# snap-research/R2L

Hardware: AMD Instinct MI355X
Metric: rays/sec (train+render) W256D88 lego@400x400 (higher is better)
Workload: dtype f32 (v_mfma_f32_32x32x2_f32: exact fp32 products and accumulate)

## Files before the change

r2l_amd/csrc/r2l_coop16.hip:

```cpp
#include "r2l_common.h"

#define C16_RAYS 16
#define C16_LD 260
#define C16_ACT_FLOATS (C16_RAYS * C16_LD)
#define C16_GROUP_BYTES (R2L_C16_GROUP_FLOATS * 4)

typedef float f32x4v __attribute__((ext_vector_type(4)));

__host__ __device__ static inline int64_t h_off_head_b() { return (int64_t)R2L_IN * R2L_W; }
__host__ __device__ static inline int64_t h_off_body_w(int layer) {
    return (int64_t)R2L_IN * R2L_W + R2L_W + (int64_t)layer * (R2L_W * R2L_W + R2L_W);
}
__host__ __device__ static inline int64_t h_off_body_b(int layer) { return h_off_body_w(layer) + R2L_W * R2L_W; }
__host__ __device__ static inline int64_t h_off_tail_w(int n_block) { return h_off_body_w(2 * n_block); }
__host__ __device__ static inline int64_t h_off_tail_b(int n_block) { return h_off_tail_w(n_block) + 3 * R2L_W; }
#define C16_BIAS_STRIDE (R2L_W * R2L_W + R2L_W)

template <int D>
struct Ring16 {
    __amdgpu_buffer_rsrc_t rsrc;
    unsigned voff;
    unsigned soff;
    f32x4 w[D][4];
    __device__ __forceinline__ f32x4 load(int t) const {
        return __builtin_bit_cast(f32x4, __builtin_amdgcn_raw_buffer_load_b128(rsrc, voff + (unsigned)t * 1024u, soff, 0));
    }
    __device__ __forceinline__ void opaque() { asm volatile("" : "+v"(voff)); }
    __device__ __forceinline__ void init(const float* stream, int64_t first_group, int lane, int wave) {
        rsrc = __builtin_amdgcn_make_buffer_rsrc(const_cast<float*>(stream), 0, 0xffffffff, 0x00020000);
        voff = (unsigned)lane * 16u + (unsigned)(4 * wave) * 1024u;
        soff = (unsigned)(first_group * C16_GROUP_BYTES);
#pragma unroll
        for (int d = 0; d < D; ++d) {
#pragma unroll
            for (int t = 0; t < 4; ++t) w[d][t] = load(t);
            soff += C16_GROUP_BYTES;
        }
    }
};

template <int SLOT, int EXTRA_RD = 0, int VPT = 0, int D>
__device__ __forceinline__ void group16(f32x4 (&acc)[4], Ring16<D>& r, const f32x4& b) {
    static_assert(SLOT >= 0 && SLOT < D, "ring slot");
    r.opaque();
#pragma unroll
    for (int e = 0; e < 3; ++e)
#pragma unroll
        for (int t = 0; t < 4; ++t) acc[t] = __builtin_amdgcn_mfma_f32_16x16x4f32(r.w[SLOT][t][e], b[e], acc[t], 0, 0, 0);
#pragma unroll
    for (int t = 0; t < 4; ++t) {
        acc[t] = __builtin_amdgcn_mfma_f32_16x16x4f32(r.w[SLOT][t][3], b[3], acc[t], 0, 0, 0);
        r.w[SLOT][t] = r.load(t);
    }
    r.soff += C16_GROUP_BYTES;
    if (EXTRA_RD > 0) __builtin_amdgcn_sched_group_barrier(0x020, EXTRA_RD, 0);
#pragma unroll
    for (int i = 0; i < 12; ++i) {
        __builtin_amdgcn_sched_group_barrier(0x008, 1, 0);
        if (VPT > 0) __builtin_amdgcn_sched_group_barrier(0x002, VPT, 0);
    }
#pragma unroll
    for (int i = 0; i < 4; ++i) {
        __builtin_amdgcn_sched_group_barrier(0x008, 1, 0);
        __builtin_amdgcn_sched_group_barrier(0x020, 1, 0);
        if (VPT > 0) __builtin_amdgcn_sched_group_barrier(0x002, VPT, 0);
    }
    __builtin_amdgcn_sched_barrier(0);
}

__device__ __forceinline__ void layer16(f32x4 (&acc)[4], const f32x4 (&bop)[16], Ring16<8>& r, const float* next_bias,
                                        f32x4 (&bn)[4]) {
#pragma unroll
    for (int t = 0; t < 4; ++t) bn[t] = *reinterpret_cast<const f32x4*>(next_bias + 16 * t);
    group16<0, 4>(acc, r, bop[0]);
    group16<1>(acc, r, bop[1]);
    group16<2>(acc, r, bop[2]);
    group16<3>(acc, r, bop[3]);
    group16<4>(acc, r, bop[4]);
    group16<5>(acc, r, bop[5]);
    group16<6>(acc, r, bop[6]);
    group16<7>(acc, r, bop[7]);
    group16<0>(acc, r, bop[8]);
    group16<1>(acc, r, bop[9]);
    group16<2>(acc, r, bop[10]);
    group16<3>(acc, r, bop[11]);
    group16<4>(acc, r, bop[12]);
    group16<5>(acc, r, bop[13]);
    group16<6>(acc, r, bop[14]);
    group16<7>(acc, r, bop[15]);
}

__device__ __forceinline__ void lds_read_bops16(const float* act, int lane, f32x4 (&bop)[16]) {
    const float* row = act + (lane & 15) * C16_LD + 4 * (lane >> 4);
#pragma unroll
    for (int G = 0; G < 16; ++G) bop[G] = *reinterpret_cast<const f32x4*>(row + 16 * G);
}
__device__ __forceinline__ void lds_write_slice16(float* act, int lane, int wave, const f32x4 (&v)[4]) {
    float* row = act + (lane & 15) * C16_LD + 64 * wave + 4 * (lane >> 4);
#pragma unroll
    for (int t = 0; t < 4; ++t) *reinterpret_cast<f32x4*>(row + 16 * t) = v[t];
}
__device__ __forceinline__ void g_store_slice16(float* base, int64_t ray, int lane, int wave, const f32x4 (&v)[4]) {
    float* row = base + ray * R2L_W + 64 * wave + 4 * (lane >> 4);
#pragma unroll
    for (int t = 0; t < 4; ++t) r2l_stash_store(row + 16 * t, v[t]);
}
__device__ __forceinline__ void g_load_slice16(const float* base, int64_t ray, int lane, int wave, f32x4 (&v)[4]) {
    const float* row = base + ray * R2L_W + 64 * wave + 4 * (lane >> 4);
#pragma unroll
    for (int t = 0; t < 4; ++t) v[t] = *reinterpret_cast<const f32x4*>(row + 16 * t);
}
__device__ __forceinline__ void rows_lds_to_global(const float* act, float* base, int64_t tile_row0, int lane, int wave) {
#pragma unroll
    for (int r = 0; r < 4; ++r) {
        const int ray = 4 * wave + r;
        const f32x4 v = *reinterpret_cast<const f32x4*>(act + ray * C16_LD + 4 * lane);
        r2l_stash_store_nt(base + (tile_row0 + ray) * R2L_W + 4 * lane, v);
    }
}
__device__ __forceinline__ float sel4(int kk, float a0, float a1, float a2, float a3) {
    const float lo = kk == 1 ? a1 : a0, hi = kk == 3 ? a3 : a2;
    return kk >= 2 ? hi : lo;
}

struct C16FwdArgs {
    const float* rays_o;
    const float* rays_d;
    const float* t_rand;
    const float* ztab;
    float c2w[12];
    int H, Wimg;
    float focal;
    const float* wstream;
    const float* params;
    int n_block;
    float* rgb;
    float* save_x;
    float* save_t;
    int64_t N;
};

template <int Gp>
__device__ __forceinline__ f32x4 trig_chunk(int kk, const float (&xb)[4]) {
    constexpr int o0 = 16 * Gp, o1 = o0 + 4, o2 = o0 + 8, o3 = o0 + 12;
    const float x = sel4(kk, xb[o0 / 20], xb[o1 / 20], xb[o2 / 20], xb[o3 / 20]);
    const float sc = sel4(kk, (float)(1 << ((o0 % 20) / 2)), (float)(1 << ((o1 % 20) / 2)), (float)(1 << ((o2 % 20) / 2)),
                          (float)(1 << ((o3 % 20) / 2)));
    f32x4 v;
    float s, c;
    r2l_sincos(x * sc, s, c);
    v[0] = s;
    v[1] = c;
    r2l_sincos(x * (sc + sc), s, c);
    v[2] = s;
    v[3] = c;
    return v;
}

template <bool POSE, bool SAVE>
__global__ __launch_bounds__(256, 1) void r2l_fwd_c16_kernel(const C16FwdArgs a) {
    __shared__ __attribute__((aligned(16))) float act[2][C16_ACT_FLOATS];
    __shared__ float tailred[4][C16_RAYS][4];
    __shared__ float zl[4][C16_RAYS][20];

    const int wave = threadIdx.x >> 6, lane = threadIdx.x & 63, j = lane & 15, kk = lane >> 4;
    const int64_t tile_row0 = (int64_t)blockIdx.x * C16_RAYS;
    const int64_t ray = tile_row0 + j;
    const bool valid = ray < a.N;
    const int64_t rc = valid ? ray : a.N - 1;
    const int64_t Np = R2L_PAD_ROWS(a.N);

    float o[3], d[3];
    if constexpr (!POSE) {
#pragma unroll
        for (int k = 0; k < 3; ++k) {
            o[k] = a.rays_o[rc * 3 + k];
            d[k] = a.rays_d[rc * 3 + k];
        }
    } else {
        const int pj = (int)(rc / a.Wimg), pi = (int)(rc % a.Wimg);
        const float dx = ((float)pi - (float)a.Wimg * 0.5f) / a.focal;
        const float dy = -(((float)pj - (float)a.H * 0.5f) / a.focal);
#pragma unroll
        for (int k = 0; k < 3; ++k) {
            d[k] = (dx * a.c2w[4 * k + 0] + dy * a.c2w[4 * k + 1]) + (-1.0f) * a.c2w[4 * k + 2];
            o[k] = a.c2w[4 * k + 3];
        }
    }
    float z[16];
#pragma unroll
    for (int q = 0; q < 4; ++q) {
        const f32x4 lo = *reinterpret_cast<const f32x4*>(a.ztab + 4 * q);
#pragma unroll
        for (int k = 0; k < 4; ++k) z[4 * q + k] = lo[k];
        if (a.t_rand != nullptr) {
            const f32x4 sp = *reinterpret_cast<const f32x4*>(a.ztab + 16 + 4 * q);
            const f32x4 u = *reinterpret_cast<const f32x4*>(a.t_rand + rc * 16 + 4 * q);
#pragma unroll
            for (int k = 0; k < 4; ++k) z[4 * q + k] = lo[k] + sp[k] * u[k];
        }
    }

    f32x4 acc[4], xo[4], x0[4], bn[4];
    {
        const float* hb = a.params + h_off_head_b() + 64 * wave + 4 * kk;
#pragma unroll
        for (int t = 0; t < 4; ++t) acc[t] = *reinterpret_cast<const f32x4*>(hb + 16 * t);
    }
    Ring16<5> r5;
    r5.init(a.wstream, 0, lane, wave);
#pragma unroll
    for (int q = 0; q < 4; ++q)
        *reinterpret_cast<f32x4*>(&zl[wave][j][4 * q]) = f32x4{z[4 * q], z[4 * q + 1], z[4 * q + 2], z[4 * q + 3]};
    auto coords = [&](int S, float (&xc)[12]) {
        const f32x4 zs = *reinterpret_cast<const f32x4*>(&zl[wave][j][4 * (S & 3)]);
#pragma unroll
        for (int i = 0; i < 12; ++i) xc[i] = o[i % 3] + d[i % 3] * zs[i / 3];
    };
    {
        float xc[12], xn[12];
        coords(0, xc);
        f32x4 cur, nxt;
        {
            const float xb[4] = {xc[0], xc[1], xc[2], xc[3]};
            cur = trig_chunk<0>(kk, xb);
        }
#define C16_HEAD_STEP(SLOT, NEXT_GP, XB)                   \
    nxt = trig_chunk<NEXT_GP>(kk, XB);                     \
    group16<SLOT, 0, 6>(acc, r5, cur);                     \
    cur = nxt;
#pragma unroll 1
        for (int S = 0; S < 4; ++S) {
            coords(S + 1, xn);
            const float b0[4] = {xc[0], xc[1], xc[2], xc[3]}, b1[4] = {xc[4], xc[5], xc[6], xc[7]};
            const float b2[4] = {xc[8], xc[9], xc[10], xc[11]}, b3[4] = {xn[0], xn[1], xn[2], xn[3]};
            C16_HEAD_STEP(0, 1, b0) C16_HEAD_STEP(1, 2, b0) C16_HEAD_STEP(2, 3, b0) C16_HEAD_STEP(3, 4, b0)
            C16_HEAD_STEP(4, 0, b1)
            C16_HEAD_STEP(0, 1, b1) C16_HEAD_STEP(1, 2, b1) C16_HEAD_STEP(2, 3, b1) C16_HEAD_STEP(3, 4, b1)
            C16_HEAD_STEP(4, 0, b2)
            C16_HEAD_STEP(0, 1, b2) C16_HEAD_STEP(1, 2, b2) C16_HEAD_STEP(2, 3, b2) C16_HEAD_STEP(3, 4, b2)
            C16_HEAD_STEP(4, 0, b3)
#pragma unroll
            for (int i = 0; i < 12; ++i) xc[i] = xn[i];
        }
#undef C16_HEAD_STEP
    }
    {
        float p[48];
#pragma unroll
        for (int c = 0; c < 48; ++c) p[c] = o[c % 3] + d[c % 3] * z[c / 3];
        f32x4 idv[3];
#pragma unroll
        for (int g = 0; g < 3; ++g)
#pragma unroll
            for (int e = 0; e < 4; ++e) idv[g][e] = sel4(kk, p[16 * g + e], p[16 * g + 4 + e], p[16 * g + 8 + e], p[16 * g + 12 + e]);
        group16<0>(acc, r5, idv[0]);
        group16<1>(acc, r5, idv[1]);
        group16<2>(acc, r5, idv[2]);
    }
#pragma unroll
    for (int t = 0; t < 4; ++t)
#pragma unroll
        for (int c = 0; c < 4; ++c) {
            xo[t][c] = fmaxf(acc[t][c], 0.f);
            x0[t][c] = xo[t][c];
        }
    lds_write_slice16(act[0], lane, wave, xo);
    Ring16<8> r8;
    r8.rsrc = r5.rsrc;
    r8.voff = r5.voff;
    r8.soff = r5.soff;
#pragma unroll
    for (int t = 0; t < 4; ++t) {
        r8.w[0][t] = r5.w[3][t];
        r8.w[1][t] = r5.w[4][t];
        r8.w[2][t] = r5.w[0][t];
        r8.w[3][t] = r5.w[1][t];
        r8.w[4][t] = r5.w[2][t];
    }
#pragma unroll
    for (int dd = 5; dd < 8; ++dd) {
#pragma unroll
        for (int t = 0; t < 4; ++t) r8.w[dd][t] = r8.load(t);
        r8.soff += C16_GROUP_BYTES;
    }

    f32x4 bop[16];
    const float* bias = a.params + h_off_body_b(0) + 64 * wave + 4 * kk;
#pragma unroll
    for (int t = 0; t < 4; ++t) bn[t] = *reinterpret_cast<const f32x4*>(bias + 16 * t);
#pragma unroll 1
    for (int b = 0; b < a.n_block; ++b) {
        __syncthreads();
        lds_read_bops16(act[0], lane, bop);
        if constexpr (SAVE) rows_lds_to_global(act[0], a.save_x + (int64_t)b * Np * R2L_W, tile_row0, lane, wave);
#pragma unroll
        for (int t = 0; t < 4; ++t) acc[t] = bn[t];
        layer16(acc, bop, r8, bias + C16_BIAS_STRIDE, bn);
#pragma unroll
        for (int t = 0; t < 4; ++t)
#pragma unroll
            for (int c = 0; c < 4; ++c) acc[t][c] = fmaxf(acc[t][c], 0.f);
        lds_write_slice16(act[1], lane, wave, acc);
        __syncthreads();
        lds_read_bops16(act[1], lane, bop);
        if constexpr (SAVE) rows_lds_to_global(act[1], a.save_t + (int64_t)b * Np * R2L_W, tile_row0, lane, wave);
#pragma unroll
        for (int t = 0; t < 4; ++t) xo[t] += bn[t];
        layer16(xo, bop, r8, b + 1 < a.n_block ? bias + 2 * C16_BIAS_STRIDE : bias, bn);
        lds_write_slice16(act[0], lane, wave, xo);
        bias += 2 * C16_BIAS_STRIDE;
    }
    if constexpr (SAVE) {
        __syncthreads();
        rows_lds_to_global(act[0], a.save_x + (int64_t)a.n_block * Np * R2L_W, tile_row0, lane, wave);
    }

    const float* tw = a.params + h_off_tail_w(a.n_block) + 64 * wave + 4 * kk;
    float p3[3] = {0.f, 0.f, 0.f};
#pragma unroll
    for (int t = 0; t < 4; ++t) {
        f32x4 wv[3];
#pragma unroll
        for (int c = 0; c < 3; ++c) wv[c] = *reinterpret_cast<const f32x4*>(tw + c * R2L_W + 16 * t);
#pragma unroll
        for (int e = 0; e < 4; ++e) {
            const float y = xo[t][e] + x0[t][e];
#pragma unroll
            for (int c = 0; c < 3; ++c) p3[c] = __builtin_fmaf(wv[c][e], y, p3[c]);
        }
    }
#pragma unroll
    for (int c = 0; c < 3; ++c) {
        p3[c] += __shfl_xor(p3[c], 16);
        p3[c] += __shfl_xor(p3[c], 32);
    }
    if (kk == 0) {
        tailred[wave][j][0] = p3[0];
        tailred[wave][j][1] = p3[1];
        tailred[wave][j][2] = p3[2];
    }
    __syncthreads();
    if (wave == 0 && kk == 0 && valid) {
#pragma unroll
        for (int c = 0; c < 3; ++c) {
            const float v = ((tailred[0][j][c] + tailred[1][j][c]) + (tailred[2][j][c] + tailred[3][j][c])) +
                            a.params[h_off_tail_b(a.n_block) + c];
            a.rgb[ray * 3 + c] = 1.0f / (1.0f + expf(-v));
        }
    }
}

struct C16BwdArgs {
    const float* rgb;
    const float* target;
    const float* drgb;
    const float* save_x;
    const float* save_t;
    const float* wstream;
    const float* params;
    int n_block;
    float grad_scale;
    float* dpre;
    float* gx;
    float* gt;
    float* sqerr_partial;
    int64_t N;
};

__device__ __forceinline__ void layer16_plain(f32x4 (&acc)[4], const f32x4 (&bop)[16], Ring16<8>& r) {
    group16<0>(acc, r, bop[0]);
    group16<1>(acc, r, bop[1]);
    group16<2>(acc, r, bop[2]);
    group16<3>(acc, r, bop[3]);
    group16<4>(acc, r, bop[4]);
    group16<5>(acc, r, bop[5]);
    group16<6>(acc, r, bop[6]);
    group16<7>(acc, r, bop[7]);
    group16<0>(acc, r, bop[8]);
    group16<1>(acc, r, bop[9]);
    group16<2>(acc, r, bop[10]);
    group16<3>(acc, r, bop[11]);
    group16<4>(acc, r, bop[12]);
    group16<5>(acc, r, bop[13]);
    group16<6>(acc, r, bop[14]);
    group16<7>(acc, r, bop[15]);
}

__global__ __launch_bounds__(256, 1) void r2l_bwd_c16_kernel(const C16BwdArgs a) {
    __shared__ __attribute__((aligned(16))) float act[2][C16_ACT_FLOATS];

    const int wave = threadIdx.x >> 6, lane = threadIdx.x & 63, j = lane & 15, kk = lane >> 4;
    const int64_t tile = blockIdx.x;
    const int64_t ray = tile * C16_RAYS + j;
    const bool valid = ray < a.N;
    const int64_t rc = valid ? ray : a.N - 1;
    const int64_t Np = R2L_PAD_ROWS(a.N);

    Ring16<8> r8;
    r8.init(a.wstream, 0, lane, wave);

    float dp[3];
#pragma unroll
    for (int c = 0; c < 3; ++c) {
        const float r = a.rgb[rc * 3 + c];
        const float dl = a.target != nullptr ? a.grad_scale * (r - a.target[rc * 3 + c]) : a.drgb[rc * 3 + c];
        dp[c] = valid ? dl * (r * (1.0f - r)) : 0.f;
    }
    if (wave == 0 && kk == 0 && valid) {
#pragma unroll
        for (int c = 0; c < 3; ++c) a.dpre[ray * 3 + c] = dp[c];
    }
    if (a.sqerr_partial != nullptr && (tile & 1) == 0 && wave == 1) {
        const int64_t r32 = tile * C16_RAYS + (lane & 31);
        float s = 0.f;
        if (a.target != nullptr && lane < 32 && r32 < a.N) {
#pragma unroll
            for (int c = 0; c < 3; ++c) {
                const float e = a.rgb[r32 * 3 + c] - a.target[r32 * 3 + c];
                s += e * e;
            }
        }
#pragma unroll
        for (int off = 32; off >= 1; off >>= 1) s += __shfl_xor(s, off);
        if (lane == 0) a.sqerr_partial[tile >> 1] = s;
    }
    f32x4 g[4], dy[4], u[4];
    {
        const float* tw = a.params + h_off_tail_w(a.n_block) + 64 * wave + 4 * kk;
#pragma unroll
        for (int t = 0; t < 4; ++t) {
            f32x4 wv[3];
#pragma unroll
            for (int c = 0; c < 3; ++c) wv[c] = *reinterpret_cast<const f32x4*>(tw + c * R2L_W + 16 * t);
#pragma unroll
            for (int e = 0; e < 4; ++e) {
                float v = wv[0][e] * dp[0];
                v = __builtin_fmaf(wv[1][e], dp[1], v);
                v = __builtin_fmaf(wv[2][e], dp[2], v);
                g[t][e] = v;
                dy[t][e] = v;
            }
        }
    }
    lds_write_slice16(act[0], lane, wave, g);

    f32x4 bop[16];
    const int64_t tile_row0 = tile * C16_RAYS;
#pragma unroll 1
    for (int b = a.n_block - 1; b >= 0; --b) {
        __syncthreads();
        lds_read_bops16(act[0], lane, bop);
        rows_lds_to_global(act[0], a.gx + (int64_t)(b + 1) * Np * R2L_W, tile_row0, lane, wave);
        f32x4 tm[4];
        g_load_slice16(a.save_t + (int64_t)b * Np * R2L_W, ray, lane, wave, tm);
#pragma unroll
        for (int t = 0; t < 4; ++t) u[t] = f32x4{0.f, 0.f, 0.f, 0.f};
        layer16_plain(u, bop, r8);
#pragma unroll
        for (int t = 0; t < 4; ++t)
#pragma unroll
            for (int c = 0; c < 4; ++c) u[t][c] = tm[t][c] > 0.f ? u[t][c] : 0.f;
        lds_write_slice16(act[1], lane, wave, u);
        __syncthreads();
        lds_read_bops16(act[1], lane, bop);
        rows_lds_to_global(act[1], a.gt + (int64_t)b * Np * R2L_W, tile_row0, lane, wave);
        layer16_plain(g, bop, r8);
        lds_write_slice16(act[0], lane, wave, g);
    }
    f32x4 xm[4];
    g_load_slice16(a.save_x, ray, lane, wave, xm);
#pragma unroll
    for (int t = 0; t < 4; ++t)
#pragma unroll
        for (int c = 0; c < 4; ++c) g[t][c] = xm[t][c] > 0.f ? g[t][c] + dy[t][c] : 0.f;
    g_store_slice16(a.gx, ray, lane, wave, g);
}

int r2l_coop16_forward(const float* rays_o, const float* rays_d, const float* t_rand, const float* ztab,
                       const float* c2w_host12, int H, int W, float focal, const float* wstream16, const float* params,
                       int n_block, float* rgb, float* save_x, float* save_t, int64_t N, hipStream_t stream) {
    C16FwdArgs a{};
    a.rays_o = rays_o; a.rays_d = rays_d; a.t_rand = t_rand; a.ztab = ztab; a.wstream = wstream16; a.params = params;
    a.n_block = n_block; a.rgb = rgb; a.save_x = save_x; a.save_t = save_t; a.N = N; a.H = H; a.Wimg = W; a.focal = focal;
    if (c2w_host12) for (int i = 0; i < 12; ++i) a.c2w[i] = c2w_host12[i];
    const dim3 grid((unsigned)(R2L_PAD_ROWS(N) / C16_RAYS)), block(256);
    if (c2w_host12) hipLaunchKernelGGL((r2l_fwd_c16_kernel<true, false>), grid, block, 0, stream, a);
    else if (save_x) hipLaunchKernelGGL((r2l_fwd_c16_kernel<false, true>), grid, block, 0, stream, a);
    else hipLaunchKernelGGL((r2l_fwd_c16_kernel<false, false>), grid, block, 0, stream, a);
    R2L_CHECK(hipGetLastError());
    return 0;
}

int r2l_coop16_backward(const float* rgb, const float* target, const float* drgb, const float* save_x,
                        const float* save_t, const float* wstream_bwd16, const float* params, int n_block,
                        float grad_scale, float* dpre, float* gx, float* gt, float* sqerr_partial, int64_t N,
                        hipStream_t stream) {
    C16BwdArgs a{};
    a.rgb = rgb; a.target = target; a.drgb = drgb; a.save_x = save_x; a.save_t = save_t; a.wstream = wstream_bwd16;
    a.params = params; a.n_block = n_block; a.grad_scale = grad_scale; a.dpre = dpre; a.gx = gx; a.gt = gt;
    a.sqerr_partial = sqerr_partial; a.N = N;
    const dim3 grid((unsigned)(R2L_PAD_ROWS(N) / C16_RAYS)), block(256);
    hipLaunchKernelGGL(r2l_bwd_c16_kernel, grid, block, 0, stream, a);
    R2L_CHECK(hipGetLastError());
    return 0;
}
```

r2l_amd/csrc/r2l_pack.hip:

```cpp
#include "r2l_dispatch.h"

__host__ __device__ static inline int64_t pk_off_body_w(int layer) {
    return (int64_t)R2L_IN * R2L_W + R2L_W + (int64_t)layer * (R2L_W * R2L_W + R2L_W);
}

__global__ void r2l_pack_fwd_kernel(const float* __restrict__ params, float* __restrict__ out, int n_block) {
    const int64_t total = (int64_t)(R2L_FWD_HEAD_GROUPS + 2 * n_block * R2L_FWD_LAYER_GROUPS) * R2L_GROUP_FLOATS;
    for (int64_t i = (int64_t)blockIdx.x * blockDim.x + threadIdx.x; i < total + R2L_STREAM_PAD;
         i += (int64_t)gridDim.x * blockDim.x) {
        if (i >= total) { out[i] = 0.f; continue; }
        const int64_t gidx = i / R2L_GROUP_FLOATS;
        const int rem = (int)(i % R2L_GROUP_FLOATS);
        const int tile = rem >> 8, lane = (rem & 255) >> 2, j = rem & 3;
        const int h = lane >> 5, o = 32 * tile + (lane & 31);
        float v;
        if (gidx < R2L_FWD_HEAD_GROUPS) {
            const int g1 = (int)gidx - 1;
            if (g1 < 0) {
                v = (j == 0 && h == 0) ? params[(int64_t)R2L_IN * R2L_W + o] : 0.f;
            } else if (g1 < R2L_HEAD_TRIG_GROUPS) {
                const int it = g1 / 15, ax = (g1 % 15) / 5, g = g1 % 5;
                const int k = ((8 * h + it) * 3 + ax) * 21 + 4 * g + j;
                v = params[(int64_t)o * R2L_IN + k];
            } else {
                const int e = 4 * (g1 - R2L_HEAD_TRIG_GROUPS) + j;
                const int k = (24 * h + e) * 21 + 20;
                v = params[(int64_t)o * R2L_IN + k];
            }
        } else {
            const int64_t gb = gidx - R2L_FWD_HEAD_GROUPS;
            const int layer = (int)(gb / R2L_FWD_LAYER_GROUPS), G = (int)(gb % R2L_FWD_LAYER_GROUPS) - 1;
            if (G < 0) {
                v = (j == 0 && h == 0) ? params[pk_off_body_w(layer) + R2L_W * R2L_W + o] : 0.f;
            } else {
                const int in = 32 * (G >> 2) + 8 * (G & 3) + 4 * h + j;
                v = params[pk_off_body_w(layer) + (int64_t)o * R2L_W + in];
            }
        }
        out[i] = v;
    }
}

__global__ void r2l_pack_bwd_kernel(const float* __restrict__ params, float* __restrict__ out, int n_block) {
    const int64_t total = (int64_t)2 * n_block * R2L_LAYER_FLOATS;
    for (int64_t i = (int64_t)blockIdx.x * blockDim.x + threadIdx.x; i < total + R2L_STREAM_PAD;
         i += (int64_t)gridDim.x * blockDim.x) {
        if (i >= total) { out[i] = 0.f; continue; }
        const int64_t gidx = i / R2L_GROUP_FLOATS;
        const int rem = (int)(i % R2L_GROUP_FLOATS);
        const int tile = rem >> 8, lane = (rem & 255) >> 2, j = rem & 3;
        const int h = lane >> 5, o = 32 * tile + (lane & 31);
        const int slot = (int)(gidx / R2L_LAYER_GROUPS), G = (int)(gidx % R2L_LAYER_GROUPS);
        const int layer = 2 * n_block - 1 - slot;
        const int in = 32 * (G >> 2) + 8 * (G & 3) + 4 * h + j;
        out[i] = params[pk_off_body_w(layer) + (int64_t)in * R2L_W + o];
    }
}

__global__ void r2l_pack_fwd16_kernel(const float* __restrict__ params, float* __restrict__ out, int n_block) {
    const int64_t total = (int64_t)(R2L_C16_HEAD_GROUPS + 2 * n_block * R2L_C16_LAYER_GROUPS) * R2L_C16_GROUP_FLOATS;
    const int64_t padded = r2l_fwd16_stream_floats(n_block);
    for (int64_t i = (int64_t)blockIdx.x * blockDim.x + threadIdx.x; i < padded; i += (int64_t)gridDim.x * blockDim.x) {
        if (i >= total) { out[i] = 0.f; continue; }
        const int64_t gidx = i / R2L_C16_GROUP_FLOATS;
        const int rem = (int)(i % R2L_C16_GROUP_FLOATS);
        const int tile = rem >> 8, lane = (rem & 255) >> 2, e = rem & 3;
        const int kk = lane >> 4, o = 16 * tile + (lane & 15);
        float v;
        if (gidx < R2L_C16_HEAD_GROUPS) {
            const int kp = 16 * (int)gidx + 4 * kk + e;
            int col;
            if (kp < 960) {
                const int B = kp / 80, off = kp % 80, ci = off / 20, slot = off % 20, f = slot >> 1;
                col = 21 * (4 * B + ci) + ((slot & 1) ? 10 + f : f);
            } else {
                col = 21 * (kp - 960) + 20;
            }
            v = params[(int64_t)o * R2L_IN + col];
        } else {
            const int64_t gb = gidx - R2L_C16_HEAD_GROUPS;
            const int layer = (int)(gb / R2L_C16_LAYER_GROUPS), G = (int)(gb % R2L_C16_LAYER_GROUPS);
            const int in = 16 * G + 4 * kk + e;
            v = params[pk_off_body_w(layer) + (int64_t)o * R2L_W + in];
        }
        out[i] = v;
    }
}

__global__ void r2l_pack_bwd16_kernel(const float* __restrict__ params, float* __restrict__ out, int n_block) {
    const int64_t total = (int64_t)2 * n_block * R2L_C16_LAYER_GROUPS * R2L_C16_GROUP_FLOATS;
    const int64_t padded = r2l_bwd16_stream_floats(n_block);
    for (int64_t i = (int64_t)blockIdx.x * blockDim.x + threadIdx.x; i < padded; i += (int64_t)gridDim.x * blockDim.x) {
        if (i >= total) { out[i] = 0.f; continue; }
        const int64_t gidx = i / R2L_C16_GROUP_FLOATS;
        const int rem = (int)(i % R2L_C16_GROUP_FLOATS);
        const int tile = rem >> 8, lane = (rem & 255) >> 2, e = rem & 3;
        const int kk = lane >> 4, o = 16 * tile + (lane & 15);
        const int slot = (int)(gidx / R2L_C16_LAYER_GROUPS), G = (int)(gidx % R2L_C16_LAYER_GROUPS);
        const int layer = 2 * n_block - 1 - slot;
        const int in = 16 * G + 4 * kk + e;
        out[i] = params[pk_off_body_w(layer) + (int64_t)in * R2L_W + o];
    }
}

extern "C" int64_t r2l_param_count(int n_block) {
    return (int64_t)R2L_IN * R2L_W + R2L_W + (int64_t)2 * n_block * (R2L_W * R2L_W + R2L_W) + 3 * R2L_W + 3;
}

extern "C" int64_t r2l_fwd_stream_floats(int n_block) {
    return r2l_fwd32_stream_floats(n_block) + r2l_fwd16_stream_floats(n_block) + r2l_fwd3_stream_floats(n_block) +
           r2l_fwd2_stream_floats(n_block);
}

extern "C" int64_t r2l_bwd_stream_floats(int n_block) {
    return r2l_bwd32_stream_floats(n_block) + r2l_bwd16_stream_floats(n_block) + r2l_bwd3_stream_floats(n_block) +
           r2l_bwd2_stream_floats(n_block);
}

extern "C" int r2l_variant_for_cfg(int64_t N, const r2l_config* cfg) {
    R2L_CFG_QUERY(cfg);
    return r2l_plan(cfg, N, 0, false, false).tiling == R2L_TILING_COOP16 ? 2 : 0;
}
extern "C" int r2l_variant_for(int64_t N) { return r2l_variant_for_cfg(N, nullptr); }
extern "C" int r2l_forward_layout_for(int64_t N, int with_stash) { return r2l_forward_layout_for_cfg(N, with_stash, nullptr); }
extern "C" int r2l_forward_layout_for_cfg(int64_t N, int with_stash, const r2l_config* cfg) {
    R2L_CFG_QUERY(cfg);
    return r2l_plan(cfg, N, 0, with_stash != 0, false).fwd_layout;
}
extern "C" int r2l_backward_layout_for(int64_t N) { return r2l_backward_layout_for_cfg(N, nullptr); }
extern "C" int r2l_backward_layout_for_cfg(int64_t N, const r2l_config* cfg) {
    R2L_CFG_QUERY(cfg);
    return r2l_plan(cfg, N, 0, true, false).bwd_layout;
}
static int pack_layouts(bool fwd, const float* params, int n_block, float* wstream, int layout, hipStream_t stream) {
    const R2LStreams w = fwd ? r2l_fwd_streams(wstream, n_block) : r2l_bwd_streams(wstream, n_block);
    if (layout == 0 || layout == 32) {
        if (fwd) hipLaunchKernelGGL(r2l_pack_fwd_kernel, dim3(2048), dim3(256), 0, stream, params, w.w32, n_block);
        else hipLaunchKernelGGL(r2l_pack_bwd_kernel, dim3(2048), dim3(256), 0, stream, params, w.w32, n_block);
        R2L_CHECK(hipGetLastError());
    }
    if (layout == 0 || layout == 16) {
        if (fwd) hipLaunchKernelGGL(r2l_pack_fwd16_kernel, dim3(2048), dim3(256), 0, stream, params, w.w16, n_block);
        else hipLaunchKernelGGL(r2l_pack_bwd16_kernel, dim3(2048), dim3(256), 0, stream, params, w.w16, n_block);
        R2L_CHECK(hipGetLastError());
    }
    if (layout == 0 || layout == 3) {
        const int rc = fwd ? r2l_fwd3_pack(params, n_block, w.w3, stream) : r2l_bwd3_pack(params, n_block, w.w3, stream);
        if (rc) return rc;
    }
    if (layout == 0 || layout == 2) {
        const int rc = fwd ? r2l_fwd2_pack(params, n_block, w.w2, stream) : r2l_bwd2_pack(params, n_block, w.w2, stream);
        if (rc) return rc;
    }
    return 0;
}
extern "C" int r2l_pack_forward_layout(const float* params, int n_block, float* wstream, int layout, void* stream) {
    R2L_REQUIRE(params && wstream, "r2l_pack_forward_layout: params / wstream is NULL");
    R2L_REQUIRE(n_block >= 0 && n_block <= R2L_MAX_BLOCKS, "r2l_pack_forward_layout: n_block out of range");
    R2L_REQUIRE(layout == 0 || layout == 32 || layout == 16 || layout == 3 || layout == 2, "r2l_pack_forward_layout: layout is 0, 32, 16, 3 or 2");
    return pack_layouts(true, params, n_block, wstream, layout, (hipStream_t)stream);
}
extern "C" int r2l_pack_backward_layout(const float* params, int n_block, float* wstream, int layout, void* stream) {
    R2L_REQUIRE(params && wstream, "r2l_pack_backward_layout: params / wstream is NULL");
    R2L_REQUIRE(n_block >= 0 && n_block <= R2L_MAX_BLOCKS, "r2l_pack_backward_layout: n_block out of range");
    R2L_REQUIRE(layout == 0 || layout == 32 || layout == 16 || layout == 3 || layout == 2, "r2l_pack_backward_layout: layout is 0, 32, 16, 3 or 2");
    return pack_layouts(false, params, n_block, wstream, layout, (hipStream_t)stream);
}

extern "C" int r2l_pack_forward(const float* params, int n_block, float* wstream, void* stream) {
    R2L_REQUIRE(params && wstream, "r2l_pack_forward: params / wstream is NULL");
    R2L_REQUIRE(n_block >= 0 && n_block <= R2L_MAX_BLOCKS, "r2l_pack_forward: n_block out of range");
    return pack_layouts(true, params, n_block, wstream, 0, (hipStream_t)stream);
}

extern "C" int r2l_pack_backward(const float* params, int n_block, float* wstream, void* stream) {
    R2L_REQUIRE(params && wstream, "r2l_pack_backward: params / wstream is NULL");
    R2L_REQUIRE(n_block >= 0 && n_block <= R2L_MAX_BLOCKS, "r2l_pack_backward: n_block out of range");
    return pack_layouts(false, params, n_block, wstream, 0, (hipStream_t)stream);
}
```

Measured before the change: 12.53 million.

## Start each layer on the wave's own activation slice before the barrier

Each wave now begins its layer GEMM on the four K-groups it produced itself, held in registers, before the __syncthreads. Only then does it read the other three waves' slices from LDS. The weight pack is rotated per wave (tile>>2) so the streamed weight order matches this own-first K ordering. Saved-activation global stores are split into an LDS read plus a deferred store issued mid-layer. The aim is to hide barrier wait and LDS read latency behind MFMA work and cut LDS traffic by a quarter, at the cost of extra registers and schedule complexity.

```diff
diff --git a/r2l_amd/csrc/r2l_coop16.hip b/r2l_amd/csrc/r2l_coop16.hip
--- a/r2l_amd/csrc/r2l_coop16.hip
+++ b/r2l_amd/csrc/r2l_coop16.hip
@@ -68,32 +68,39 @@
     __builtin_amdgcn_sched_barrier(0);
 }
 
-__device__ __forceinline__ void layer16(f32x4 (&acc)[4], const f32x4 (&bop)[16], Ring16<8>& r, const float* next_bias,
-                                        f32x4 (&bn)[4]) {
-#pragma unroll
-    for (int t = 0; t < 4; ++t) bn[t] = *reinterpret_cast<const f32x4*>(next_bias + 16 * t);
-    group16<0, 4>(acc, r, bop[0]);
-    group16<1>(acc, r, bop[1]);
-    group16<2>(acc, r, bop[2]);
-    group16<3>(acc, r, bop[3]);
-    group16<4>(acc, r, bop[4]);
-    group16<5>(acc, r, bop[5]);
-    group16<6>(acc, r, bop[6]);
-    group16<7>(acc, r, bop[7]);
-    group16<0>(acc, r, bop[8]);
-    group16<1>(acc, r, bop[9]);
-    group16<2>(acc, r, bop[10]);
-    group16<3>(acc, r, bop[11]);
-    group16<4>(acc, r, bop[12]);
-    group16<5>(acc, r, bop[13]);
-    group16<6>(acc, r, bop[14]);
-    group16<7>(acc, r, bop[15]);
-}
-
-__device__ __forceinline__ void lds_read_bops16(const float* act, int lane, f32x4 (&bop)[16]) {
+template <int EXTRA_RD = 0>
+__device__ __forceinline__ void layer16_own01(f32x4 (&acc)[4], const f32x4 (&src)[4], Ring16<8>& r) {
+    group16<0, EXTRA_RD>(acc, r, src[0]);
+    group16<1>(acc, r, src[1]);
+}
+template <class F>
+__device__ __forceinline__ void layer16_rest(f32x4 (&acc)[4], const f32x4 (&src)[4], const f32x4 (&bop)[12], Ring16<8>& r,
+                                             F after2) {
+    group16<2>(acc, r, src[2]);
+    after2();
+    group16<3>(acc, r, src[3]);
+    group16<4>(acc, r, bop[0]);
+    group16<5>(acc, r, bop[1]);
+    group16<6>(acc, r, bop[2]);
+    group16<7>(acc, r, bop[3]);
+    group16<0>(acc, r, bop[4]);
+    group16<1>(acc, r, bop[5]);
+    group16<2>(acc, r, bop[6]);
+    group16<3>(acc, r, bop[7]);
+    group16<4>(acc, r, bop[8]);
+    group16<5>(acc, r, bop[9]);
+    group16<6>(acc, r, bop[10]);
+    group16<7>(acc, r, bop[11]);
+}
+
+__device__ __forceinline__ void lds_read_foreign16(const float* act, int lane, int wave, f32x4 (&bop)[12]) {
     const float* row = act + (lane & 15) * C16_LD + 4 * (lane >> 4);
 #pragma unroll
-    for (int G = 0; G < 16; ++G) bop[G] = *reinterpret_cast<const f32x4*>(row + 16 * G);
+    for (int q = 0; q < 3; ++q) {
+        const float* fw = row + 64 * ((wave + 1 + q) & 3);
+#pragma unroll
+        for (int t = 0; t < 4; ++t) bop[4 * q + t] = *reinterpret_cast<const f32x4*>(fw + 16 * t);
+    }
 }
 __device__ __forceinline__ void lds_write_slice16(float* act, int lane, int wave, const f32x4 (&v)[4]) {
     float* row = act + (lane & 15) * C16_LD + 64 * wave + 4 * (lane >> 4);
@@ -117,6 +124,14 @@
         const f32x4 v = *reinterpret_cast<const f32x4*>(act + ray * C16_LD + 4 * lane);
         r2l_stash_store_nt(base + (tile_row0 + ray) * R2L_W + 4 * lane, v);
     }
+}
+__device__ __forceinline__ void rows_lds_read(const float* act, int lane, int wave, f32x4 (&rv)[4]) {
+#pragma unroll
+    for (int r = 0; r < 4; ++r) rv[r] = *reinterpret_cast<const f32x4*>(act + (4 * wave + r) * C16_LD + 4 * lane);
+}
+__device__ __forceinline__ void rows_store_global(const f32x4 (&rv)[4], float* base, int64_t tile_row0, int lane, int wave) {
+#pragma unroll
+    for (int r = 0; r < 4; ++r) r2l_stash_store_nt(base + (tile_row0 + 4 * wave + r) * R2L_W + 4 * lane, rv[r]);
 }
 __device__ __forceinline__ float sel4(int kk, float a0, float a1, float a2, float a3) {
     const float lo = kk == 1 ? a1 : a0, hi = kk == 3 ? a3 : a2;
@@ -285,29 +300,42 @@
         r8.soff += C16_GROUP_BYTES;
     }
 
-    f32x4 bop[16];
+    f32x4 bop[12], rv[4];
     const float* bias = a.params + h_off_body_b(0) + 64 * wave + 4 * kk;
 #pragma unroll
     for (int t = 0; t < 4; ++t) bn[t] = *reinterpret_cast<const f32x4*>(bias + 16 * t);
 #pragma unroll 1
     for (int b = 0; b < a.n_block; ++b) {
+#pragma unroll
+        for (int t = 0; t < 4; ++t) acc[t] = bn[t];
+#pragma unroll
+        for (int t = 0; t < 4; ++t) bn[t] = *reinterpret_cast<const f32x4*>(bias + C16_BIAS_STRIDE + 16 * t);
+        layer16_own01<4>(acc, xo, r8);
         __syncthreads();
-        lds_read_bops16(act[0], lane, bop);
-        if constexpr (SAVE) rows_lds_to_global(act[0], a.save_x + (int64_t)b * Np * R2L_W, tile_row0, lane, wave);
-#pragma unroll
-        for (int t = 0; t < 4; ++t) acc[t] = bn[t];
-        layer16(acc, bop, r8, bias + C16_BIAS_STRIDE, bn);
+        lds_read_foreign16(act[0], lane, wave, bop);
+        if constexpr (SAVE) rows_lds_read(act[0], lane, wave, rv);
+        layer16_rest(acc, xo, bop, r8, [&] {
+            if constexpr (SAVE) rows_store_global(rv, a.save_x + (int64_t)b * Np * R2L_W, tile_row0, lane, wave);
+        });
 #pragma unroll
         for (int t = 0; t < 4; ++t)
 #pragma unroll
             for (int c = 0; c < 4; ++c) acc[t][c] = fmaxf(acc[t][c], 0.f);
         lds_write_slice16(act[1], lane, wave, acc);
+#pragma unroll
+        for (int t = 0; t < 4; ++t) xo[t] += bn[t];
+        {
+            const float* nb = b + 1 < a.n_block ? bias + 2 * C16_BIAS_STRIDE : bias;
+#pragma unroll
+            for (int t = 0; t < 4; ++t) bn[t] = *reinterpret_cast<const f32x4*>(nb + 16 * t);
+        }
+        layer16_own01<4>(xo, acc, r8);
         __syncthreads();
-        lds_read_bops16(act[1], lane, bop);
-        if constexpr (SAVE) rows_lds_to_global(act[1], a.save_t + (int64_t)b * Np * R2L_W, tile_row0, lane, wave);
-#pragma unroll
-        for (int t = 0; t < 4; ++t) xo[t] += bn[t];
-        layer16(xo, bop, r8, b + 1 < a.n_block ? bias + 2 * C16_BIAS_STRIDE : bias, bn);
+        lds_read_foreign16(act[1], lane, wave, bop);
+        if constexpr (SAVE) rows_lds_read(act[1], lane, wave, rv);
+        layer16_rest(xo, acc, bop, r8, [&] {
+            if constexpr (SAVE) rows_store_global(rv, a.save_t + (int64_t)b * Np * R2L_W, tile_row0, lane, wave);
+        });
         lds_write_slice16(act[0], lane, wave, xo);
         bias += 2 * C16_BIAS_STRIDE;
     }
@@ -368,25 +396,6 @@
     int64_t N;
 };
 
-__device__ __forceinline__ void layer16_plain(f32x4 (&acc)[4], const f32x4 (&bop)[16], Ring16<8>& r) {
-    group16<0>(acc, r, bop[0]);
-    group16<1>(acc, r, bop[1]);
-    group16<2>(acc, r, bop[2]);
-    group16<3>(acc, r, bop[3]);
-    group16<4>(acc, r, bop[4]);
-    group16<5>(acc, r, bop[5]);
-    group16<6>(acc, r, bop[6]);
-    group16<7>(acc, r, bop[7]);
-    group16<0>(acc, r, bop[8]);
-    group16<1>(acc, r, bop[9]);
-    group16<2>(acc, r, bop[10]);
-    group16<3>(acc, r, bop[11]);
-    group16<4>(acc, r, bop[12]);
-    group16<5>(acc, r, bop[13]);
-    group16<6>(acc, r, bop[14]);
-    group16<7>(acc, r, bop[15]);
-}
-
 __global__ __launch_bounds__(256, 1) void r2l_bwd_c16_kernel(const C16BwdArgs a) {
     __shared__ __attribute__((aligned(16))) float act[2][C16_ACT_FLOATS];
 
@@ -445,27 +454,33 @@
     }
     lds_write_slice16(act[0], lane, wave, g);
 
-    f32x4 bop[16];
+    f32x4 bop[12], rv[4];
     const int64_t tile_row0 = tile * C16_RAYS;
 #pragma unroll 1
     for (int b = a.n_block - 1; b >= 0; --b) {
+#pragma unroll
+        for (int t = 0; t < 4; ++t) u[t] = f32x4{0.f, 0.f, 0.f, 0.f};
+        layer16_own01(u, g, r8);
         __syncthreads();
-        lds_read_bops16(act[0], lane, bop);
-        rows_lds_to_global(act[0], a.gx + (int64_t)(b + 1) * Np * R2L_W, tile_row0, lane, wave);
+        lds_read_foreign16(act[0], lane, wave, bop);
+        rows_lds_read(act[0], lane, wave, rv);
         f32x4 tm[4];
         g_load_slice16(a.save_t + (int64_t)b * Np * R2L_W, ray, lane, wave, tm);
-#pragma unroll
-        for (int t = 0; t < 4; ++t) u[t] = f32x4{0.f, 0.f, 0.f, 0.f};
-        layer16_plain(u, bop, r8);
+        layer16_rest(u, g, bop, r8, [&] {
+            rows_store_global(rv, a.gx + (int64_t)(b + 1) * Np * R2L_W, tile_row0, lane, wave);
+        });
 #pragma unroll
         for (int t = 0; t < 4; ++t)
 #pragma unroll
             for (int c = 0; c < 4; ++c) u[t][c] = tm[t][c] > 0.f ? u[t][c] : 0.f;
         lds_write_slice16(act[1], lane, wave, u);
+        layer16_own01(g, u, r8);
         __syncthreads();
-        lds_read_bops16(act[1], lane, bop);
-        rows_lds_to_global(act[1], a.gt + (int64_t)b * Np * R2L_W, tile_row0, lane, wave);
-        layer16_plain(g, bop, r8);
+        lds_read_foreign16(act[1], lane, wave, bop);
+        rows_lds_read(act[1], lane, wave, rv);
+        layer16_rest(g, u, bop, r8, [&] {
+            rows_store_global(rv, a.gt + (int64_t)b * Np * R2L_W, tile_row0, lane, wave);
+        });
         lds_write_slice16(act[0], lane, wave, g);
     }
     f32x4 xm[4];
diff --git a/r2l_amd/csrc/r2l_pack.hip b/r2l_amd/csrc/r2l_pack.hip
--- a/r2l_amd/csrc/r2l_pack.hip
+++ b/r2l_amd/csrc/r2l_pack.hip
@@ -79,7 +79,8 @@
             v = params[(int64_t)o * R2L_IN + col];
         } else {
             const int64_t gb = gidx - R2L_C16_HEAD_GROUPS;
-            const int layer = (int)(gb / R2L_C16_LAYER_GROUPS), G = (int)(gb % R2L_C16_LAYER_GROUPS);
+            const int layer = (int)(gb / R2L_C16_LAYER_GROUPS), pos = (int)(gb % R2L_C16_LAYER_GROUPS);
+            const int G = (4 * (tile >> 2) + pos) & 15;
             const int in = 16 * G + 4 * kk + e;
             v = params[pk_off_body_w(layer) + (int64_t)o * R2L_W + in];
         }
@@ -96,8 +97,9 @@
         const int rem = (int)(i % R2L_C16_GROUP_FLOATS);
         const int tile = rem >> 8, lane = (rem & 255) >> 2, e = rem & 3;
         const int kk = lane >> 4, o = 16 * tile + (lane & 15);
-        const int slot = (int)(gidx / R2L_C16_LAYER_GROUPS), G = (int)(gidx % R2L_C16_LAYER_GROUPS);
+        const int slot = (int)(gidx / R2L_C16_LAYER_GROUPS), pos = (int)(gidx % R2L_C16_LAYER_GROUPS);
         const int layer = 2 * n_block - 1 - slot;
+        const int G = (4 * (tile >> 2) + pos) & 15;
         const int in = 16 * G + 4 * kk + e;
         out[i] = params[pk_off_body_w(layer) + (int64_t)in * R2L_W + o];
     }
```

Result: no change. 12.53 million (median of 2 runs) (+0.1%).
